# ShudaLi/rgbd_pose_estimation

Hardware: AMD Instinct MI355X
Metric: correspondence-residuals/sec (higher is better)
Workload: dtype f32; 1 GPU; configs[1]: 640x480 dense depth, 307200 3D-3D corr, point-to-point GN step (K1 normal eq + host 6x6 solve + SE3 exp) over inlier mask; corr_rank0=307200, global_corr=307200, collective=none, rccl_ranks=0, rccl_verified=False, repeats=1

## Files before the change

rgbd_pose_estimation_amd/csrc/rpe_normal_eq.hip:

```cpp
#include "rpe_residuals.hpp"

namespace rpe {

__global__ void gn_update_probe_kernel(const double* __restrict__ rec, double* __restrict__ pose, double* __restrict__ step_ok,
                                       double rel_floor) {
  __shared__ double s_rec[32];
  __shared__ double s_pose[12];
  if (threadIdx.x < 32) s_rec[threadIdx.x] = rec[threadIdx.x];
  if (threadIdx.x < 12) s_pose[threadIdx.x] = pose[threadIdx.x];
  __syncthreads();
  if (threadIdx.x == 0) {
    double step = 0.0;
    const bool ok = gn_solve_update<0>(s_rec, s_pose, &step, rel_floor);
    step_ok[0] = step; step_ok[1] = ok ? 1.0 : 0.0;
    if (ok) for (int k = 0; k < 12; k++) pose[k] = s_pose[k];
  }
}
hipError_t launch_gn_update_probe(const double* d_rec, double* d_pose, double* d_step_ok, double pivot_floor, hipStream_t s) {
  hipLaunchKernelGGL(gn_update_probe_kernel, dim3(1), dim3(64), 0, s, d_rec, d_pose, d_step_ok, pivot_floor);
  return hipGetLastError();
}

template <class T, int KIND, int BLK, bool MASK, bool WEIGHT, bool CLEAN>
__global__ __launch_bounds__(BLK) void normal_eq_kernel(const T* __restrict__ xw, const T* __restrict__ b, const T* __restrict__ c,
// ... 28 lines not shown
#pragma unroll
  for (int k = 0; k < NACC; k++) carry[k] = V2{T(0), T(0)};
  int carried = 0;
  int64_t g = (int64_t)blockIdx.x * BLK + threadIdx.x;
  V a0, a1, a2, b0, b1, b2, c0, c1, c2;
  short m[P];
  T wv[P];
  if (g < full) {
    a0 = xw4[3 * g]; a1 = xw4[3 * g + 1]; a2 = xw4[3 * g + 2];
    b0 = b4[3 * g]; b1 = b4[3 * g + 1]; b2 = b4[3 * g + 2];
    if (KIND == KIND_P2PLANE) { c0 = c4[3 * g]; c1 = c4[3 * g + 1]; c2 = c4[3 * g + 2]; }
    if (MASK) load_mask_full(mask, g, m);
    if (WEIGHT) load_weight_full(weight, g, wv);
    pin16(a0); pin16(a1); pin16(a2); pin16(b0); pin16(b1); pin16(b2);
    if (KIND == KIND_P2PLANE) { pin16(c0); pin16(c1); pin16(c2); }
  }
#if defined(RPE_STAMPS) && RPE_STAMPS >= 2
  asm volatile("s_waitcnt vmcnt(0)" ::: "memory");
  RPE_STAMP(11);
#endif
  while (g < full) {
    const int64_t gn = g + stride;
    const int64_t gl = gn < full ? gn : g;
    const V na0 = xw4[3 * gl], na1 = xw4[3 * gl + 1], na2 = xw4[3 * gl + 2];
    const V nb0 = b4[3 * gl], nb1 = b4[3 * gl + 1], nb2 = b4[3 * gl + 2];
    V nc0, nc1, nc2;
    if (KIND == KIND_P2PLANE) { nc0 = c4[3 * gl]; nc1 = c4[3 * gl + 1]; nc2 = c4[3 * gl + 2]; }
    short nm[P];
    T nwv[P];
    if (MASK) load_mask_full(mask, gl, nm);
    if (WEIGHT) load_weight_full(weight, gl, nwv);
    __builtin_amdgcn_sched_barrier(0);
    T vw[3 * P], vb[3 * P], vc[3 * P];
    unpack3(a0, a1, a2, vw);
    unpack3(b0, b1, b2, vb);
    if (KIND == KIND_P2PLANE) unpack3(c0, c1, c2, vc);
    pair_group<T, KIND, MASK, WEIGHT, CLEAN, NACC>(pose, vw, vb, vc, m, wv, P, carry);
    if (++carried == kShare) { flush_pairs<T, NACC>(carry, acc); carried = 0; }
    a0 = na0; a1 = na1; a2 = na2; b0 = nb0; b1 = nb1; b2 = nb2;
    if (KIND == KIND_P2PLANE) { c0 = nc0; c1 = nc1; c2 = nc2; }
    __builtin_amdgcn_sched_barrier(0);
    pin16(a0); pin16(a1); pin16(a2); pin16(b0); pin16(b1); pin16(b2);
    if (KIND == KIND_P2PLANE) { pin16(c0); pin16(c1); pin16(c2); }
#pragma unroll
    for (int i = 0; i < P; i++) { if (MASK) m[i] = nm[i]; if (WEIGHT) wv[i] = nwv[i]; }
    g = gn;
  }
  if (blockIdx.x == 0 && threadIdx.x == 0 && full * P < n) {
    T vw[3 * P], vb[3 * P], vc[3 * P];
    short lm[P];
    T lwv[P];
    load_group<T>(xw, full, n, vw);
    load_group<T>(b, full, n, vb);
    if (KIND == KIND_P2PLANE) load_group<T>(c, full, n, vc);
    if (MASK) load_scalars<T, short>(mask, full, n, lm, (short)0);
    if (WEIGHT) load_scalars<T, T>(weight, full, n, lwv, T(0));
    pair_group<T, KIND, MASK, WEIGHT, CLEAN, NACC>(pose, vw, vb, vc, lm, lwv, (int)(n - full * P), carry);
    carried = 1;
  }
  if (carried) flush_pairs<T, NACC>(carry, acc);
  RPE_STAMP(1);
  reduce_and_finish<NACC, kNeLd, KIND == KIND_P2P ? 1 : 0, BLK>(acc, fin);
}

template <class T, int KIND, int BLK, bool MASK, bool WEIGHT, int NREG, int AUTO, bool CLEAN>
__global__ __launch_bounds__(BLK) void normal_eq_resident_kernel(const T* __restrict__ xw, const T* __restrict__ b, const T* __restrict__ c,
                             const short* __restrict__ mask, const T* __restrict__ weight, int64_t n,
                             const unsigned long long* __restrict__ ctl, unsigned long long first_tag, int max_iters, Finish fin) {
  constexpr int P = Pk<T>::P;
  constexpr int NACC = KIND == KIND_P2P ? 17 : 29;
  constexpr bool IN_REGS = NREG > 0;
  constexpr int GPT = IN_REGS ? NREG : 1;
  __shared__ double s_pose[12];
  __shared__ int s_go;
  const int64_t full = n / P, groups = (n + P - 1) / P;
  constexpr bool with_solver = AUTO == 2;
  const int workers = (int)gridDim.x;
  const int64_t stride = (int64_t)workers * BLK;
  const int64_t g0 = (int64_t)blockIdx.x * (BLK * GPT) + threadIdx.x;
  T rw[GPT][3 * P], rb[GPT][3 * P], rc[GPT][3 * P];
  short rm[GPT][P];
  T rwv[GPT][P];
  int rpresent[GPT];
#pragma unroll
  for (int r = 0; r < GPT; r++) {
    rpresent[r] = 0;
    const int64_t g = g0 + (int64_t)r * BLK;
    if (IN_REGS && g < groups) {
      load_any_group<T, KIND, MASK, WEIGHT>(xw, b, c, mask, weight, g, full, n, rw[r], rb[r], rc[r], rm[r], rwv[r]);
      rpresent[r] = g < full ? P : (int)(n - full * P);
    }
  }
#ifdef RPE_SOLVER_DEBUG
  if (with_solver && threadIdx.x == 0) __hip_atomic_store(solver_pose_area(fin, workers, NACC) + 32 + blockIdx.x, wall_clock64(), __ATOMIC_RELAXED, __HIP_MEMORY_SCOPE_AGENT);
#endif
  constexpr bool autonomous = AUTO != 0;
  double tol = 0.0;
  if (autonomous) {
    if (threadIdx.x < 12) s_pose[threadIdx.x] = fin.gn_pose[threadIdx.x];
    tol = fin.gn->tol;
    __syncthreads();
  }
  for (int it = 1; it <= max_iters; it++) {
    if (!autonomous && resident_wait_pose<BLK>(ctl, first_tag + (unsigned long long)it, s_pose, &s_go,
        fin.pose_wait_ticks) != 1) return;
    if (with_solver && it > 1 && solver_wait_pose<BLK>(solver_pose_area(fin, workers, NACC), first_tag + (unsigned long long)it, s_pose, &s_go, it == 2 ? kSolverMeetTicks : 200000000ull) != 0) return;
#ifdef RPE_STAMPS
    const bool stamp_it = it == 1000;
    if (stamp_it) RPE_STAMP(0);
#endif
    PoseK<double> pose;
#pragma unroll
    for (int k = 0; k < 9; k++) pose.R[k] = s_pose[k];
#pragma unroll
    for (int k = 0; k < 3; k++) pose.t[k] = s_pose[9 + k];
    double acc[NACC];
#pragma unroll
    for (int k = 0; k < NACC; k++) acc[k] = 0.0;
    if (IN_REGS) {
#pragma unroll
      for (int r = 0; r < GPT; r++)
        if (rpresent[r] > 0) normal_eq_group<T, KIND, MASK, WEIGHT, NACC, CLEAN>(pose, rw[r], rb[r], rc[r], rm[r], rwv[r], rpresent[r], acc);
    } else {
      for (int64_t g = g0; g < groups; g += stride) {
        T vw[3 * P], vb[3 * P], vc[3 * P];
        short mm[P];
        T ww[P];
        load_any_group<T, KIND, MASK, WEIGHT>(xw, b, c, mask, weight, g, full, n, vw, vb, vc, mm, ww);
        normal_eq_group<T, KIND, MASK, WEIGHT, NACC, CLEAN>(pose, vw, vb, vc, mm, ww, g < full ? P : (int)(n - full * P), acc);
      }
    }
#ifdef RPE_STAMPS
    if (stamp_it) RPE_STAMP(1);
#endif
#ifndef RPE_STAMPS
    const bool stamp_it = false;
#endif
    if (with_solver) { solver_send_sums<NACC, BLK>(acc, fin, first_tag + (unsigned long long)it); continue; }
    if (autonomous) {
      if (resident_auto_stage<NACC, BLK>(acc, fin, first_tag + (unsigned long long)it, it, max_iters, tol, s_pose,
          stamp_it) != 0) return;
      continue;
    }
    if (!resident_cross_stage<NACC, BLK>(acc, fin, first_tag + (unsigned long long)it, fin.seq + (unsigned long long)it,
        stamp_it)) return;
  }
}

#ifdef RPE_STAMPS
}
extern "C" int rpe_debug_read_stamps(unsigned long long* out, int nwords) {
  if (nwords > 4096 * 16) nwords = 4096 * 16;
  if (hipDeviceSynchronize() != hipSuccess) return -1;
  if (hipMemcpyFromSymbol(out, HIP_SYMBOL(rpe::g_stamps), (size_t)nwords * 8) != hipSuccess) return -1;
  static unsigned long long zeros[4096 * 16];
  return hipMemcpyToSymbol(HIP_SYMBOL(rpe::g_stamps), zeros, sizeof(zeros)) == hipSuccess ? 0 : -1;
}
namespace rpe {
#endif

template <int MODE>
__global__ __launch_bounds__(64) void chain_finish_kernel(const double* __restrict__ runs, const double* __restrict__ pose_in, GnState* st,
                                                          double rel_floor, double* __restrict__ h_pairs, unsigned long long seq) {
  __shared__ double f_tot[32];
  __shared__ double f_pose[12];
  __shared__ double f_out[16];
  if (threadIdx.x < 12) f_pose[threadIdx.x] = pose_in[threadIdx.x];
  if (threadIdx.x < 32) {
    double t = 0.0;
#pragma unroll
    for (int r = 0; r < kRunSlots; r++) t += runs[r * kRunLd + threadIdx.x];
    f_tot[threadIdx.x] = t;
  }
  __syncthreads();
  if (threadIdx.x == 0) {
    double step = st->step;
    bool ok = st->status == 0;
    if (!st->done) ok = gn_solve_update<MODE>(f_tot, f_pose, &step, rel_floor);
    for (int k = 0; k < 12; k++) f_out[k] = f_pose[k];
    f_out[12] = step; f_out[13] = st->done ? st->cost : record_entry<MODE>(f_tot, 27); f_out[14] = (double)(st->iters + (st->done ? 0 : 1));
    f_out[15] = ok ? 0.0 : 1.0;
  }
  __syncthreads();
  if (threadIdx.x < 16) store_tagged_pair(h_pairs, threadIdx.x, f_out[threadIdx.x], seq);
}
hipError_t launch_chain_finish(int kind, const double* d_runs, const double* d_pose, GnState* d_state, double pivot_floor, double* h_pairs,
                               unsigned long long seq, hipStream_t s) {
  if (kind == KIND_P2P) hipLaunchKernelGGL((chain_finish_kernel<1>), dim3(1), dim3(64), 0, s, d_runs, d_pose, d_state, pivot_floor, h_pairs, seq);
  else hipLaunchKernelGGL((chain_finish_kernel<0>), dim3(1), dim3(64), 0, s, d_runs, d_pose, d_state, pivot_floor, h_pairs, seq);
  return hipGetLastError();
}

template <class T, int KIND, int BLK>
static void normal_eq_launch(const DeviceArrays& A, int flags, const PoseK<double>& pose, const ReduceTarget& rt, hipStream_t s,
                             hipEvent_t ev0, hipEvent_t ev1) {
  const T* xw = (const T*)A.a[0];
  const T* b = (const T*)((KIND == KIND_BEARING || KIND == KIND_REPROJ) ? A.a[2] : A.a[1]);
  const T* c = (const T*)A.a[4];
  const int mod = (KIND == KIND_BEARING || KIND == KIND_REPROJ) ? 0 : 1;
  const short* mask = (flags & F_USE_MASK) ? A.mask[mod] : nullptr;
  const T* weight = (flags & F_USE_WEIGHT) ? (const T*)A.weight[mod] : nullptr;
  const int G = reduce_grid(A.n, Pk<T>::P, rt.max_blocks, BLK);
  const Finish fin = make_finish(rt);
#define RPE_NE_LAUNCH2(M, W, C) RPE_LAUNCH_EV((normal_eq_kernel<T, KIND, BLK, M, W, C>), dim3(G), dim3(BLK), 0, s, ev0, ev1, xw, b, c, mask, weight, A.n, pose, fin)
#define RPE_NE_LAUNCH(M, W) do { if constexpr (sizeof(T) == 4) { if (rt.clean) { RPE_NE_LAUNCH2(M, W, true); break; } } RPE_NE_LAUNCH2(M, W, false); } while (0)
  if (mask && weight) RPE_NE_LAUNCH(true, true);
  else if (mask) RPE_NE_LAUNCH(true, false);
  else if (weight) RPE_NE_LAUNCH(false, true);
  else RPE_NE_LAUNCH(false, false);
#undef RPE_NE_LAUNCH
#undef RPE_NE_LAUNCH2
}
template <class T>
static hipError_t normal_eq_t(const DeviceArrays& A, int kind, int flags, const double* pose12, const ReduceTarget& rt, hipStream_t s,
                              hipEvent_t ev0, hipEvent_t ev1) {
  const PoseK<double> pose = make_pose<double>(pose12);
  const int blk = (sizeof(T) == 8 && kind != KIND_P2P) ? 256 : pick_block(rt);
  if (kind == KIND_P2P) {
    if (blk == 512) normal_eq_launch<T, KIND_P2P, 512>(A, flags, pose, rt, s, ev0, ev1);
    else normal_eq_launch<T, KIND_P2P, 256>(A, flags, pose, rt, s, ev0, ev1);
  } else if (kind == KIND_P2PLANE) {
    if (blk == 512) { if constexpr (sizeof(T) == 4) normal_eq_launch<T, KIND_P2PLANE, 512>(A, flags, pose, rt, s, ev0, ev1); }
    else normal_eq_launch<T, KIND_P2PLANE, 256>(A, flags, pose, rt, s, ev0, ev1);
  } else if (kind == KIND_BEARING) {
    if (blk == 512) { if constexpr (sizeof(T) == 4) normal_eq_launch<T, KIND_BEARING, 512>(A, flags, pose, rt, s, ev0, ev1); }
    else normal_eq_launch<T, KIND_BEARING, 256>(A, flags, pose, rt, s, ev0, ev1);
  } else if (kind == KIND_REPROJ) {
    if (blk == 512) { if constexpr (sizeof(T) == 4) normal_eq_launch<T, KIND_REPROJ, 512>(A, flags, pose, rt, s, ev0, ev1); }
// ... 130 lines not shown
```

rgbd_pose_estimation_amd/csrc/rpe_residuals.hpp:

```cpp
#pragma once
#include "rpe_reduce.hpp"

namespace rpe {

template <class C> __device__ __forceinline__ void add_row(const C (&J)[6], C r, C w, C (&s)[29]) {
  int k = 0;
#pragma unroll
  for (int a = 0; a < 6; a++) {
    const C wa = w * J[a];
#pragma unroll
    for (int b = a; b < 6; b++) { s[k] = fma(wa, J[b], s[k]); k++; }
    s[21 + a] = fma(wa, r, s[21 + a]);
  }
  s[27] = fma(w * r, r, s[27]);
}
template <class V> __device__ __forceinline__ void add_row2(const V (&J)[6], V r, V w, V (&s)[29]) {
  int k = 0;
#pragma unroll
  for (int a = 0; a < 6; a++) {
    const V wa = w * J[a];
#pragma unroll
    for (int b = a; b < 6; b++) { s[k] = __builtin_elementwise_fma(wa, J[b], s[k]); k++; }
    s[21 + a] = __builtin_elementwise_fma(wa, r, s[21 + a]);
  }
// ... 107 lines not shown
  w = ok ? w : C(0);
  n1 = ok ? (C)fma(pxd, (double)bz, -(double)bx * pzd) : C(0);
  n2 = ok ? (C)fma(pyd, (double)bz, -(double)by * pzd) : C(0);
  px = ok ? (C)pxd : C(0); py = ok ? (C)pyd : C(0); pz = ok ? (C)pzd : C(1);
  bzs = ok ? bz : C(1);
}
template <class C>
__device__ __forceinline__ void reproj_pair(const PoseK<double>& T, const C (&x)[2], const C (&y)[2], const C (&z)[2], const C (&bx)[2],
                                            const C (&by)[2], const C (&bz)[2], const C (&w)[2], C __attribute__((ext_vector_type(2))) (&s)[29]) {
  typedef C V __attribute__((ext_vector_type(2)));
  C px[2], py[2], pz[2], n1[2], n2[2], bzs[2], wi[2];
#pragma unroll
  for (int e = 0; e < 2; e++) {
    double pxd, pyd, pzd;
    transform<C>(T, x[e], y[e], z[e], pxd, pyd, pzd);
    wi[e] = w[e];
    reproj_prepare<C>(pxd, pyd, pzd, bx[e], by[e], bz[e], wi[e], px[e], py[e], pz[e], n1[e], n2[e], bzs[e]);
  }
  reproj_rows<V>(V{px[0], px[1]}, V{py[0], py[1]}, V{pz[0], pz[1]}, V{n1[0], n1[1]}, V{n2[0], n2[1]}, V{bzs[0], bzs[1]},
                 V{wi[0], wi[1]}, V{wi[0], wi[1]}, s);
}
template <class C>
__device__ __forceinline__ void reproj_point(double pxd, double pyd, double pzd, C bx, C by, C bz, C w, C w_count, C (&s)[29]) {
  C px, py, pz, n1, n2, bzs, wc = w_count;
  reproj_prepare<C>(pxd, pyd, pzd, bx, by, bz, wc, px, py, pz, n1, n2, bzs);
  reproj_rows<C>(px, py, pz, n1, n2, bzs, wc == C(0) ? C(0) : w, wc, s);
}
template <class C>
__device__ __forceinline__ C reproj_residual_norm(double pxd, double pyd, double pzd, C bx, C by, C bz) {
  if (!(pzd > kReprojMinZ && (double)bz > kReprojMinZ)) return C(0);
  const double r1 = pxd / pzd - (double)bx / (double)bz, r2 = pyd / pzd - (double)by / (double)bz;
  return (C)sqrt(r1 * r1 + r2 * r2);
}
template <class C>
__device__ __forceinline__ void bearing_pair(const PoseK<double>& T, const C (&x)[2], const C (&y)[2], const C (&z)[2], const C (&bx)[2],
                                             const C (&by)[2], const C (&bz)[2], const C (&w)[2],
                                             C __attribute__((ext_vector_type(2))) (&s)[29]) {
  typedef C V __attribute__((ext_vector_type(2)));
  const V BX = {bx[0], bx[1]}, BY = {by[0], by[1]}, BZ = {bz[0], bz[1]};
  V e1[3], e2[3];
  tangent_basis<V>(BX, BY, BZ, e1, e2);
  C px[2], py[2], pz[2], d1[2], d2[2];
#pragma unroll
  for (int e = 0; e < 2; e++) {
    double pxd, pyd, pzd;
    transform<C>(T, x[e], y[e], z[e], pxd, pyd, pzd);
    px[e] = (C)pxd; py[e] = (C)pyd; pz[e] = (C)pzd;
    d1[e] = (C)dot_e_p(e1[0][e], e1[1][e], e1[2][e], pxd, pyd, pzd);
    d2[e] = (C)dot_e_p(e2[0][e], e2[1][e], e2[2][e], pxd, pyd, pzd);
  }
  bearing_rows<V>(V{px[0], px[1]}, V{py[0], py[1]}, V{pz[0], pz[1]}, e1, e2, V{d1[0], d1[1]}, V{d2[0], d2[1]}, BX, BY, BZ,
      V{w[0], w[1]},
                  V{w[0], w[1]}, s);
}


template <class V> __device__ __forceinline__ void p2p_accumulate(V px, V py, V pz, V rx, V ry, V rz, V w, V (&s)[17]) {
  const V wpx = w * px, wpy = w * py, wpz = w * pz;
  const V wrx = w * rx, wry = w * ry, wrz = w * rz;
  s[0] += w;
  s[1] += wpx; s[2] += wpy; s[3] += wpz;
  s[4] = __builtin_elementwise_fma(wpx, px, s[4]); s[5] = __builtin_elementwise_fma(wpx, py, s[5]);
  s[6] = __builtin_elementwise_fma(wpx, pz, s[6]); s[7] = __builtin_elementwise_fma(wpy, py, s[7]);
  s[8] = __builtin_elementwise_fma(wpy, pz, s[8]); s[9] = __builtin_elementwise_fma(wpz, pz, s[9]);
  s[10] += wrx; s[11] += wry; s[12] += wrz;
  s[13] += py * wrz - pz * wry;
  s[14] += pz * wrx - px * wrz;
  s[15] += px * wry - py * wrx;
  s[16] = __builtin_elementwise_fma(wrx, rx, __builtin_elementwise_fma(wry, ry, __builtin_elementwise_fma(wrz, rz, s[16])));
}
template <class C>
__device__ __forceinline__ void p2p_pair(const PoseK<double>& T, const C (&x)[2], const C (&y)[2], const C (&z)[2], const C (&cx)[2],
                                         const C (&cy)[2], const C (&cz)[2], const C (&w)[2], C __attribute__((ext_vector_type(2))) (&s)[17]) {
  typedef C V __attribute__((ext_vector_type(2)));
  C px[2], py[2], pz[2], rx[2], ry[2], rz[2];
#pragma unroll
  for (int e = 0; e < 2; e++) {
    double pxd, pyd, pzd;
    transform<C>(T, x[e], y[e], z[e], pxd, pyd, pzd);
    px[e] = (C)pxd; py[e] = (C)pyd; pz[e] = (C)pzd;
    rx[e] = (C)(pxd - (double)cx[e]); ry[e] = (C)(pyd - (double)cy[e]); rz[e] = (C)(pzd - (double)cz[e]);
  }
  p2p_accumulate<V>(V{px[0], px[1]}, V{py[0], py[1]}, V{pz[0], pz[1]}, V{rx[0], rx[1]}, V{ry[0], ry[1]}, V{rz[0], rz[1]}, V{w[0], w[1]}, s);
}

template <class T, int KIND, bool MASK, bool WEIGHT, bool CLEAN, int NS>
__device__ __forceinline__ void pair_group(const PoseK<double>& pose, const T (&vw)[3 * Pk<T>::P], const T (&vb)[3 * Pk<T>::P],
                                           const T (&vc)[3 * Pk<T>::P], const short (&m)[Pk<T>::P], const T (&wv)[Pk<T>::P],
                                           int npresent, T __attribute__((ext_vector_type(2))) (&s2)[NS]) {
  constexpr int P = Pk<T>::P;
  static_assert(NS == (KIND == KIND_P2P ? 17 : 29), "sums per kind");
  static_assert(KIND == KIND_P2P || KIND == KIND_P2PLANE || KIND == KIND_BEARING || KIND == KIND_REPROJ, "residual kinds");
#pragma unroll
  for (int j = 0; j < P / 2; j++) {
    T x[2], y[2], z[2], bx[2], by[2], bz[2], nx[2], ny[2], nz[2], wi[2];
#pragma unroll
    for (int e = 0; e < 2; e++) {
      const int i = 2 * j + e;
      bx[e] = vb[3 * i]; by[e] = vb[3 * i + 1]; bz[e] = vb[3 * i + 2];
      T w = WEIGHT ? wv[i] : T(1);
      if (MASK) w = m[i] == 1 ? w : T(0);
      if (CLEAN) {
        w = i < npresent ? w : T(0);
        x[e] = vw[3 * i]; y[e] = vw[3 * i + 1]; z[e] = vw[3 * i + 2];
        if (KIND == KIND_P2PLANE) { nx[e] = vc[3 * i]; ny[e] = vc[3 * i + 1]; nz[e] = vc[3 * i + 2]; }
      } else {
        w = (i < npresent && !all_nan(bx[e], by[e], bz[e])) ? w : T(0);
        const bool off = w == T(0);
        x[e] = off ? T(0) : vw[3 * i]; y[e] = off ? T(0) : vw[3 * i + 1];
        z[e] = off ? ((KIND == KIND_BEARING || KIND == KIND_REPROJ) ? T(1) : T(0)) : vw[3 * i + 2];
        bx[e] = off ? T(0) : bx[e]; by[e] = off ? T(0) : by[e]; bz[e] = off ? T(1) : bz[e];
        if (KIND == KIND_P2PLANE) { nx[e] = off ? T(0) : vc[3 * i]; ny[e] = off ? T(0) : vc[3 * i + 1];
            nz[e] = off ? T(0) : vc[3 * i + 2]; }
      }
      wi[e] = w;
    }
    if constexpr (KIND == KIND_P2P) p2p_pair<T>(pose, x, y, z, bx, by, bz, wi, s2);
    else if constexpr (KIND == KIND_P2PLANE) p2plane_pair<T>(pose, x, y, z, bx, by, bz, nx, ny, nz, wi, s2);
    else if constexpr (KIND == KIND_BEARING) bearing_pair<T>(pose, x, y, z, bx, by, bz, wi, s2);
    else {
      reproj_pair<T>(pose, x, y, z, bx, by, bz, wi, s2);
      if (CLEAN) {
        typedef T V __attribute__((ext_vector_type(2)));
        const V all = ((V{x[0], x[1]} + V{y[0], y[1]}) + (V{z[0], z[1]} + V{bx[0], bx[1]})) + (V{by[0], by[1]} + V{bz[0], bz[1]});
        s2[27] = __builtin_elementwise_fma(V{T(0), T(0)}, all, s2[27]);
      }
    }
  }
}
template <class T, int NS>
__device__ __forceinline__ void flush_pairs(T __attribute__((ext_vector_type(2))) (&s2)[NS], double (&acc)[NS]) {
  typedef T V __attribute__((ext_vector_type(2)));
#pragma unroll
  for (int k = 0; k < NS; k++) { acc[k] += (double)(s2[k].x + s2[k].y); s2[k] = V{T(0), T(0)}; }
}

template <class T, int KIND, bool MASK, bool WEIGHT, int NACC, bool CLEAN = false>
__device__ __forceinline__ void normal_eq_group(const PoseK<double>& pose, const T (&vw)[3 * Pk<T>::P], const T (&vb)[3 * Pk<T>::P],
                                                const T (&vc)[3 * Pk<T>::P], const short (&m)[Pk<T>::P], const T (&wv)[Pk<T>::P],
                                                int npresent, double (&acc)[NACC]) {
  typedef T V __attribute__((ext_vector_type(2)));
  V s2[NACC];
#pragma unroll
  for (int k = 0; k < NACC; k++) s2[k] = V{T(0), T(0)};
  pair_group<T, KIND, MASK, WEIGHT, CLEAN, NACC>(pose, vw, vb, vc, m, wv, npresent, s2);
  flush_pairs<T, NACC>(s2, acc);
}
constexpr unsigned long long kResidentStop = 1ull << 63;
template <class T, int KIND, bool MASK, bool WEIGHT>
__device__ __forceinline__ void load_any_group(const T* __restrict__ xw, const T* __restrict__ b, const T* __restrict__ c,
                                               const short* __restrict__ mask, const T* __restrict__ weight, int64_t g, int64_t full,
                                               int64_t n, T (&vw)[3 * Pk<T>::P], T (&vb)[3 * Pk<T>::P], T (&vc)[3 * Pk<T>::P],
                                               short (&m)[Pk<T>::P], T (&wv)[Pk<T>::P]) {
  typedef typename Pk<T>::V V;
  if (g < full) {
    const V* xw4 = reinterpret_cast<const V*>(xw);
    const V* b4 = reinterpret_cast<const V*>(b);
    const V x0 = xw4[3 * g], x1 = xw4[3 * g + 1], x2 = xw4[3 * g + 2];
    const V y0 = b4[3 * g], y1 = b4[3 * g + 1], y2 = b4[3 * g + 2];
    unpack3(x0, x1, x2, vw);
    unpack3(y0, y1, y2, vb);
    if (KIND == KIND_P2PLANE) { const V* c4 = reinterpret_cast<const V*>(c);
        const V z0 = c4[3 * g], z1 = c4[3 * g + 1], z2 = c4[3 * g + 2]; unpack3(z0, z1, z2, vc); }
    if (MASK) load_mask_full(mask, g, m);
    if (WEIGHT) load_weight_full(weight, g, wv);
  } else {
// ... 4 lines not shown
    if (WEIGHT) load_scalars<T, T>(weight, g, n, wv, T(0));
  }
}

constexpr int kAutoMaxRunSums = 1024;
__device__ __forceinline__ int resident_judge_pose(unsigned long long w, unsigned long long want) {
  const unsigned int lo = (unsigned int)w, hi = (unsigned int)(w >> 32);
  const unsigned long long ta = ((unsigned long long)__builtin_amdgcn_readlane(hi, 0) << 32) | __builtin_amdgcn_readlane(lo, 0);
  const unsigned long long tb = ((unsigned long long)__builtin_amdgcn_readlane(hi, 15) << 32) | __builtin_amdgcn_readlane(lo, 15);
  if (ta != tb) return 0;
  const unsigned long long num = ta & ~kResidentStop;
  if (num == want) return (ta & kResidentStop) ? 2 : 1;
  return num > want ? 2 : 0;
}
template <int BLK>
__device__ __forceinline__ int resident_wait_pose(const unsigned long long* __restrict__ ctl, unsigned long long want,
                                                  double* __restrict__ s_pose, int* __restrict__ s_go,
                                                  unsigned long long wait_ticks = 200000000ull) {
  if (threadIdx.x < 64) {
    const int lane = threadIdx.x;
    const unsigned long long t0 = wall_clock64();
    int go = 0;
    unsigned long long w = 0;
    for (;;) {
      if (lane < 16) w = __hip_atomic_load(ctl + lane, __ATOMIC_RELAXED, __HIP_MEMORY_SCOPE_SYSTEM);
      if ((go = resident_judge_pose(w, want)) != 0) break;
      if (wall_clock64() - t0 > wait_ticks) { go = 3; break; }
      __builtin_amdgcn_s_sleep(2);
    }
    if (lane >= 1 && lane <= 12) s_pose[lane - 1] = __longlong_as_double((long long)w);
    if (lane == 0) *s_go = go;
  }
  __syncthreads();
  return *s_go;
}
struct RunShape { int run, row, leader, rows, runs, step; };
__device__ __forceinline__ RunShape run_shape(const Finish& fin, int G) {
  RunShape s;
  const int b = (int)blockIdx.x;
  if (fin.stride > 1) {
    const int S = fin.stride < G ? fin.stride : G;
    s.run = b % S; s.row = b / S; s.leader = s.run; s.rows = (G - s.run + S - 1) / S; s.runs = S; s.step = S;
  } else {
    const int R = fin.rows;
    s.run = b / R; s.leader = s.run * R; s.row = b - s.leader; s.rows = min(R, G - s.leader); s.runs = (G + R - 1) / R; s.step = 1;
  }
  return s;
}
template <int NACC, int BLK>
__device__ __forceinline__ bool resident_cross_own(double own, const Finish& fin, unsigned long long tag, unsigned long long seq, bool stamp_it) {
  constexpr int RGN = BLK / NACC;
  __shared__ double g_part[RGN][NACC];
  unsigned long long* gran = reinterpret_cast<unsigned long long*>(fin.partials);
  const RunShape rs = run_shape(fin, (int)gridDim.x);
  const int run = rs.run, leader = rs.leader;
  if ((int)blockIdx.x != leader) {
    const bool withheld = fin.fault_tag != 0 && tag == fin.fault_tag && blockIdx.x + 1 == gridDim.x;
    if (threadIdx.x < NACC && !withheld) store_granule16(gran + 2 * ((size_t)blockIdx.x * NACC + threadIdx.x), own, tag);
#ifdef RPE_STAMPS
    if (stamp_it) RPE_STAMP(2);
#endif
    return true;
  }
  if (threadIdx.x < NACC) g_part[0][threadIdx.x] = own;
#ifdef RPE_STAMPS
  if (stamp_it) RPE_STAMP(2);
#endif
  const int rows = rs.rows;
  const bool lost = collect_rows<NACC, BLK>(gran, (int)gridDim.x, leader, rows, tag, g_part, rs.step);
#ifdef RPE_STAMPS
  if (stamp_it) RPE_STAMP(3);
#endif
  const bool ok = !__syncthreads_or(lost);
#ifdef RPE_STAMPS
  if (stamp_it) RPE_STAMP(4);
#endif
  if (threadIdx.x < NACC) store_tagged_pair(fin.out_host, run * NACC + threadIdx.x,
      ok ? sum_rows_lane<NACC, RGN>(g_part, rows < RGN ? rows : RGN, threadIdx.x) : __longlong_as_double((long long)kLostMarker), seq);
#ifdef RPE_STAMPS
  if (stamp_it) RPE_STAMP(5);
#endif
  return ok;
}
template <int NACC, int BLK>
__device__ __forceinline__ bool resident_cross_stage(const double (&acc)[NACC], const Finish& fin, unsigned long long tag,
                                                     unsigned long long seq, bool stamp_it) {
  constexpr int NW = BLK / 64;
  __shared__ double g_red[NW][NACC];
  const int lane = threadIdx.x & 63, wave = threadIdx.x >> 6;
  wave_reduce_to<NACC>(acc, g_red[wave], lane);
  __syncthreads();
  double own = 0.0;
  if (threadIdx.x < NACC) {
#pragma unroll
    for (int w = 0; w < NW; w++) own += g_red[w][threadIdx.x];
  }
  return resident_cross_own<NACC, BLK>(own, fin, tag, seq, stamp_it);
}

template <int NACC, int BLK>
__device__ __forceinline__ int resident_auto_stage(const double (&acc)[NACC], const Finish& fin, unsigned long long tag, int it,
                                                   int max_iters, double tol, double* __restrict__ s_pose, bool stamp_it = false) {
  constexpr int NW = BLK / 64;
  constexpr int RGN = BLK / NACC;
  constexpr int MODE = NACC == 17 ? 1 : 0;
  __shared__ double a_red[NW][NACC];
  __shared__ double a_part[RGN][NACC];
  __shared__ double a_runs[kAutoMaxRunSums];
  __shared__ double a_tot[32];
  __shared__ double a_step;
  __shared__ int a_ok;
  const int lane = threadIdx.x & 63, wave = threadIdx.x >> 6;
  const int G = (int)gridDim.x;
  const RunShape rs = run_shape(fin, G);
  const int run = rs.run, leader = rs.leader, runs = rs.runs;
  unsigned long long* gran = reinterpret_cast<unsigned long long*>(fin.partials);
  unsigned long long* rrec = gran + 2 * ((size_t)G * NACC + (size_t)(it & 1) * runs * NACC);
  wave_reduce_to<NACC>(acc, a_red[wave], lane);
  __syncthreads();
  if (threadIdx.x < NACC) {
    double own = 0.0;
#pragma unroll
    for (int w = 0; w < NW; w++) own += a_red[w][threadIdx.x];
    if ((int)blockIdx.x != leader) store_granule16(gran + 2 * ((size_t)blockIdx.x * NACC + threadIdx.x), own, tag);
    else a_part[0][threadIdx.x] = own;
  }
#ifdef RPE_STAMPS
  if (stamp_it) RPE_STAMP(2);
#endif
  bool lost = runs * NACC > kAutoMaxRunSums;
  if (!lost && (int)blockIdx.x == leader) {
    const int rows = rs.rows;
    lost = __syncthreads_or(collect_rows<NACC, BLK>(gran, G, leader, rows, tag, a_part, rs.step));
    if (!lost) {
      const double t = sum_rows<NACC, BLK>(a_part, rows < RGN ? rows : RGN);
      if (threadIdx.x < NACC) { if (G == 1) a_runs[threadIdx.x] = t; else store_granule16(rrec + 2 * ((size_t)run * NACC + threadIdx.x), t, tag); }
    }
  }
#ifdef RPE_STAMPS
  if (stamp_it) RPE_STAMP(3);
#endif
  if (!lost && G > 1) {
    const int total = runs * NACC;
    for (int i = threadIdx.x; i < total; i += BLK) {
      const unsigned long long t0 = wall_clock64();
      granule_t q;
      for (unsigned int spins = 1;; spins++) {
        q = load_granule16(rrec + 2 * (size_t)i);
        if ((((unsigned long long)q.w << 32) | q.z) == tag) break;
        if ((spins & 63u) == 0 && wall_clock64() - t0 > 200000000ull) { lost = true; break; }
      }
      a_runs[i] = __longlong_as_double((long long)(((unsigned long long)q.y << 32) | q.x));
    }
  }
  lost = __syncthreads_or(lost);
#ifdef RPE_STAMPS
  if (stamp_it) RPE_STAMP(4);
#endif
  if (threadIdx.x < 64) {
    if (!lost) {
      double t = 0.0;
      if (threadIdx.x < NACC) for (int r = 0; r < runs; r++) t += a_runs[r * NACC + threadIdx.x];
      if (threadIdx.x < 32) a_tot[threadIdx.x] = threadIdx.x < NACC ? t : 0.0;
    }
    __builtin_amdgcn_fence(__ATOMIC_RELEASE, "wavefront");
    __builtin_amdgcn_wave_barrier();
    __builtin_amdgcn_fence(__ATOMIC_ACQUIRE, "wavefront");
#ifdef RPE_STAMPS
    if (stamp_it) RPE_STAMP(5);
#endif
    if (threadIdx.x == 0) {
      double step = 0.0;
      a_ok = !lost && gn_solve_update<MODE>(a_tot, s_pose, &step, fin.pivot_floor) ? 1 : 0;
      a_step = step;
    }
  }
  __syncthreads();
#ifdef RPE_STAMPS
  if (stamp_it) RPE_STAMP(6);
#endif
  const bool ok = a_ok != 0;
  const bool done = !ok || a_step < tol || it >= max_iters;
  if (done && blockIdx.x == 0 && threadIdx.x == 0 && fin.out_host) {
    for (int k = 0; k < 12; k++) __hip_atomic_store(fin.out_host + k, s_pose[k], __ATOMIC_RELAXED, __HIP_MEMORY_SCOPE_SYSTEM);
    __hip_atomic_store(fin.out_host + 12, a_step, __ATOMIC_RELAXED, __HIP_MEMORY_SCOPE_SYSTEM);
    __hip_atomic_store(fin.out_host + 13, lost ? 0.0 : record_entry<MODE>(a_tot, 27), __ATOMIC_RELAXED, __HIP_MEMORY_SCOPE_SYSTEM);
    __hip_atomic_store(fin.out_host + 14, (double)it, __ATOMIC_RELAXED, __HIP_MEMORY_SCOPE_SYSTEM);
    __hip_atomic_store(fin.out_host + 15, ok ? 0.0 : (lost ? 2.0 : 1.0), __ATOMIC_RELAXED, __HIP_MEMORY_SCOPE_SYSTEM);
    __hip_atomic_store(fin.out_host + 16, lost ? 0.0 : record_entry<MODE>(a_tot, 28), __ATOMIC_RELAXED, __HIP_MEMORY_SCOPE_SYSTEM);
    asm volatile("s_waitcnt vmcnt(0)" ::: "memory");
    __hip_atomic_store(reinterpret_cast<unsigned long long*>(fin.out_host + 32), fin.seq, __ATOMIC_RELAXED, __HIP_MEMORY_SCOPE_SYSTEM);
  }
  return lost ? 2 : (done ? 1 : 0);
}

constexpr int kSolverPoseGranules = 14;
constexpr unsigned long long kSolverMeetTicks = 25000000ull;
__device__ __forceinline__ unsigned long long* solver_pose_area(const Finish& fin, int workers, int nacc) {
  return reinterpret_cast<unsigned long long*>(fin.partials) + 2 * ((size_t)(workers + 8) * nacc);
}
template <int BLK>
__device__ __forceinline__ int solver_wait_pose(const unsigned long long* __restrict__ area, unsigned long long want, double* __restrict__ s_pose,
                                                int* __restrict__ s_go, unsigned long long wait_ticks = 200000000ull) {
  if (threadIdx.x < 64) {
    const int lane = threadIdx.x;
    const unsigned long long t0 = wall_clock64();
    granule_t q = {};
    int go = -1;
    for (unsigned int spins = 1;; spins++) {
      bool have = true;
      if (lane < kSolverPoseGranules) {
        q = load_granule16(area + 2 * (size_t)lane);
        have = (((unsigned long long)q.w << 32) | q.z) == want;
      }
      if (__builtin_amdgcn_ballot_w64(!have) == 0) { go = 0; break; }
      if ((spins & 63u) == 0 && wall_clock64() - t0 > wait_ticks) { go = 3; break; }
      __builtin_amdgcn_s_sleep(1);
    }
    const double v = __longlong_as_double((long long)(((unsigned long long)q.y << 32) | q.x));
    if (lane < 12) s_pose[lane] = v;
    if (lane == 13) *s_go = go == 3 ? 3 : (int)v;
  }
  __syncthreads();
  return *s_go;
}
template <int NACC, int BLK>
__device__ __forceinline__ void solver_send_sums(const double (&acc)[NACC], const Finish& fin, unsigned long long tag) {
  constexpr int NW = BLK / 64;
  __shared__ double w_red[NW][NACC];
  const int lane = threadIdx.x & 63, wave = threadIdx.x >> 6;
  unsigned long long* gran = reinterpret_cast<unsigned long long*>(fin.partials);
  wave_reduce_to<NACC>(acc, w_red[wave], lane);
  __syncthreads();
  if (threadIdx.x < NACC) {
    double own = 0.0;
#pragma unroll
    for (int w = 0; w < NW; w++) own += w_red[w][threadIdx.x];
    store_granule16(gran + 2 * ((size_t)blockIdx.x * NACC + threadIdx.x), own, tag);
  }
  __syncthreads();
}
template <int NACC, int BLK>
__device__ __forceinline__ void solver_loop(const Finish& fin, int workers, unsigned long long first_tag, int max_iters) {
  constexpr int RGN = BLK / NACC;
  constexpr int MODE = NACC == 17 ? 1 : 0;
  __shared__ double v_part[RGN][NACC];
  __shared__ double v_tot[32];
  __shared__ double v_pose[12];
  __shared__ double v_step;
  __shared__ int v_code;
  unsigned long long* gran = reinterpret_cast<unsigned long long*>(fin.partials);
  unsigned long long* area = solver_pose_area(fin, workers, NACC);
#ifdef RPE_SOLVER_DEBUG
  const unsigned long long dbg_start = wall_clock64();
#endif
  if (threadIdx.x < 12) v_pose[threadIdx.x] = fin.gn_pose[threadIdx.x];
  const double tol = fin.gn->tol;
  __syncthreads();
  for (int it = 1; it <= max_iters; it++) {
    const unsigned long long tag = first_tag + (unsigned long long)it;
    if (threadIdx.x < NACC) v_part[0][threadIdx.x] = 0.0;
    __syncthreads();
    bool lost = collect_rows<NACC, BLK, 12>(gran, workers, -1, workers + 1, tag, v_part, 1, it <= 2 ? kSolverMeetTicks : 200000000ull);
    lost = __syncthreads_or(lost);
    if (lost && threadIdx.x == 0 && fin.out_host) {
      int missing = 0, lo = workers, hi = -1;
      for (int w = 0; w < workers; w++) {
        const granule_t q = load_granule16(gran + 2 * ((size_t)w * NACC + NACC - 1));
        if ((((unsigned long long)q.w << 32) | q.z) != tag) { missing++; lo = w < lo ? w : lo; hi = w; }
      }
#ifdef RPE_SOLVER_DEBUG
      {
        unsigned long long mn = ~0ull, mx = 0; int started = 0;
        for (int w = 0; w < workers; w++) {
          const unsigned long long v = __hip_atomic_load(area + 32 + w, __ATOMIC_RELAXED, __HIP_MEMORY_SCOPE_AGENT);
          if (v > dbg_start - 100000000ull) { started++; mn = v < mn ? v : mn; mx = v > mx ? v : mx; }
        }
        __hip_atomic_store(fin.out_host + 20, (double)started, __ATOMIC_RELAXED, __HIP_MEMORY_SCOPE_SYSTEM);
        __hip_atomic_store(fin.out_host + 21, started ? ((double)mn - (double)dbg_start) * 0.01 : -1.0, __ATOMIC_RELAXED, __HIP_MEMORY_SCOPE_SYSTEM);
        __hip_atomic_store(fin.out_host + 22, started ? ((double)mx - (double)dbg_start) * 0.01 : -1.0, __ATOMIC_RELAXED, __HIP_MEMORY_SCOPE_SYSTEM);
        __hip_atomic_store(fin.out_host + 23, ((double)wall_clock64() - (double)dbg_start) * 0.01, __ATOMIC_RELAXED, __HIP_MEMORY_SCOPE_SYSTEM);
      }
#endif
      __hip_atomic_store(fin.out_host + 17, (double)missing, __ATOMIC_RELAXED, __HIP_MEMORY_SCOPE_SYSTEM);
      __hip_atomic_store(fin.out_host + 18, (double)lo, __ATOMIC_RELAXED, __HIP_MEMORY_SCOPE_SYSTEM);
      __hip_atomic_store(fin.out_host + 19, (double)hi, __ATOMIC_RELAXED, __HIP_MEMORY_SCOPE_SYSTEM);
    }
    const double t = sum_rows<NACC, BLK>(v_part, workers + 1 < RGN ? workers + 1 : RGN);
    if (threadIdx.x < 64) {
      if (threadIdx.x < 32) v_tot[threadIdx.x] = threadIdx.x < NACC ? t : 0.0;
      __builtin_amdgcn_fence(__ATOMIC_RELEASE, "wavefront");
      __builtin_amdgcn_wave_barrier();
      __builtin_amdgcn_fence(__ATOMIC_ACQUIRE, "wavefront");
      if (threadIdx.x == 0) {
        double step = 0.0;
        const bool ok = !lost && gn_solve_update<MODE>(v_tot, v_pose, &step, fin.pivot_floor);
        v_step = step;
        v_code = !ok ? 2 : ((step < tol || it >= max_iters) ? 1 : 0);
      }
      __builtin_amdgcn_fence(__ATOMIC_RELEASE, "wavefront");
      __builtin_amdgcn_wave_barrier();
      __builtin_amdgcn_fence(__ATOMIC_ACQUIRE, "wavefront");
      const int lane = threadIdx.x;
      if (lane == 0 && v_code != 0 && fin.out_host) {
        const bool ok = v_code == 1;
        for (int k = 0; k < 12; k++) __hip_atomic_store(fin.out_host + k, v_pose[k], __ATOMIC_RELAXED, __HIP_MEMORY_SCOPE_SYSTEM);
        __hip_atomic_store(fin.out_host + 12, v_step, __ATOMIC_RELAXED, __HIP_MEMORY_SCOPE_SYSTEM);
        __hip_atomic_store(fin.out_host + 13, lost ? 0.0 : record_entry<MODE>(v_tot, 27), __ATOMIC_RELAXED, __HIP_MEMORY_SCOPE_SYSTEM);
        __hip_atomic_store(fin.out_host + 14, (double)it, __ATOMIC_RELAXED, __HIP_MEMORY_SCOPE_SYSTEM);
        __hip_atomic_store(fin.out_host + 15, ok ? 0.0 : (lost ? 2.0 : 1.0), __ATOMIC_RELAXED, __HIP_MEMORY_SCOPE_SYSTEM);
        __hip_atomic_store(fin.out_host + 16, lost ? 0.0 : record_entry<MODE>(v_tot, 28), __ATOMIC_RELAXED, __HIP_MEMORY_SCOPE_SYSTEM);
        asm volatile("s_waitcnt vmcnt(0)" ::: "memory");
        __hip_atomic_store(reinterpret_cast<unsigned long long*>(fin.out_host + 32), fin.seq, __ATOMIC_RELAXED, __HIP_MEMORY_SCOPE_SYSTEM);
        asm volatile("s_waitcnt vmcnt(0)" ::: "memory");
      }
      __builtin_amdgcn_fence(__ATOMIC_RELEASE, "wavefront");
      __builtin_amdgcn_wave_barrier();
      if (lane < kSolverPoseGranules) {
        const double v = lane < 12 ? v_pose[lane] : (lane == 12 ? v_step : (double)v_code);
        store_granule16(area + 2 * (size_t)lane, v, tag + 1);
// ... 17 lines not shown
```

Baseline: 45.72 billion correspondence-residuals/s.

## Precompute sanitised weights and pose-invariant weight sum once in resident P2P kernel

For the register-resident f32 point-to-point path, the mask/weight/NaN sanitisation is done once before the iteration loop, and the weight sum (accumulator 0, which does not depend on the pose) is reduced once and reused every iteration. The per-iteration loop then uses a dedicated packed-f32 accumulation over register groups and a 16-wide wave reduce-scatter in place of reducing all 17 sums. This cuts per-iteration ALU and reduction work, at the cost of extra registers for the precomputed weights and some code duplication across three staging paths.

Measured after the change: 48.23 billion correspondence-residuals/s, median of 6. +5.5%, better.

```diff
diff --git a/rgbd_pose_estimation_amd/csrc/rpe_normal_eq.hip b/rgbd_pose_estimation_amd/csrc/rpe_normal_eq.hip
--- a/rgbd_pose_estimation_amd/csrc/rpe_normal_eq.hip
+++ b/rgbd_pose_estimation_amd/csrc/rpe_normal_eq.hip
@@ -134,6 +134,9 @@
   short rm[GPT][P];
   T rwv[GPT][P];
   int rpresent[GPT];
+  constexpr bool ONCE = IN_REGS && KIND == KIND_P2P && sizeof(T) == 4;
+  T rwt[GPT][P];
+  double sum0 = 0.0;
 #pragma unroll
   for (int r = 0; r < GPT; r++) {
     rpresent[r] = 0;
@@ -141,8 +144,15 @@
     if (IN_REGS && g < groups) {
       load_any_group<T, KIND, MASK, WEIGHT>(xw, b, c, mask, weight, g, full, n, rw[r], rb[r], rc[r], rm[r], rwv[r]);
       rpresent[r] = g < full ? P : (int)(n - full * P);
+    } else if (ONCE) {
+#pragma unroll
+      for (int k = 0; k < 3 * P; k++) { rw[r][k] = T(0); rb[r][k] = T(0); }
+#pragma unroll
+      for (int k = 0; k < P; k++) { rm[r][k] = 0; rwv[r][k] = T(0); }
     }
-  }
+    if constexpr (ONCE) resident_sanitise<T, MASK, WEIGHT, CLEAN>(rw[r], rb[r], rm[r], rwv[r], rpresent[r], rwt[r]);
+  }
+  if constexpr (ONCE) sum0 = resident_weight_sum<T, GPT, BLK>(rwt);
 #ifdef RPE_SOLVER_DEBUG
   if (with_solver && threadIdx.x == 0) __hip_atomic_store(solver_pose_area(fin, workers, NACC) + 32 + blockIdx.x, wall_clock64(), __ATOMIC_RELAXED, __HIP_MEMORY_SCOPE_AGENT);
 #endif
@@ -167,6 +177,23 @@
 #pragma unroll
     for (int k = 0; k < 3; k++) pose.t[k] = s_pose[9 + k];
     double acc[NACC];
+    if constexpr (ONCE) {
+      p2p_groups_in_regs<T, GPT>(pose, rw, rb, rwt, acc);
+#ifdef RPE_STAMPS
+      if (stamp_it) RPE_STAMP(1);
+#endif
+#ifndef RPE_STAMPS
+      const bool stamp_it = false;
+#endif
+      if (with_solver) { solver_send_sums<NACC, BLK, true>(acc, fin, first_tag + (unsigned long long)it, sum0); continue; }
+      if (autonomous) {
+        if (resident_auto_stage<NACC, BLK, true>(acc, fin, first_tag + (unsigned long long)it, it, max_iters, tol, s_pose,
+            stamp_it, sum0) != 0) return;
+        continue;
+      }
+      if (!resident_cross_stage<NACC, BLK, true>(acc, fin, first_tag + (unsigned long long)it, fin.seq + (unsigned long long)it,
+          stamp_it, sum0)) return;
+    } else {
 #pragma unroll
     for (int k = 0; k < NACC; k++) acc[k] = 0.0;
     if (IN_REGS) {
@@ -196,6 +223,7 @@
     }
     if (!resident_cross_stage<NACC, BLK>(acc, fin, first_tag + (unsigned long long)it, fin.seq + (unsigned long long)it,
         stamp_it)) return;
+    }
   }
 }
 
diff --git a/rgbd_pose_estimation_amd/csrc/rpe_residuals.hpp b/rgbd_pose_estimation_amd/csrc/rpe_residuals.hpp
--- a/rgbd_pose_estimation_amd/csrc/rpe_residuals.hpp
+++ b/rgbd_pose_estimation_amd/csrc/rpe_residuals.hpp
@@ -213,6 +213,84 @@
     rx[e] = (C)(pxd - (double)cx[e]); ry[e] = (C)(pyd - (double)cy[e]); rz[e] = (C)(pzd - (double)cz[e]);
   }
   p2p_accumulate<V>(V{px[0], px[1]}, V{py[0], py[1]}, V{pz[0], pz[1]}, V{rx[0], rx[1]}, V{ry[0], ry[1]}, V{rz[0], rz[1]}, V{w[0], w[1]}, s);
+}
+template <class T, int NG>
+__device__ __forceinline__ void p2p_groups_in_regs(const PoseK<double>& pose, const T (&vw)[NG][3 * Pk<T>::P],
+                                                   const T (&vb)[NG][3 * Pk<T>::P], const T (&w)[NG][Pk<T>::P], double (&acc)[17]) {
+  constexpr int P = Pk<T>::P;
+  typedef T V __attribute__((ext_vector_type(2)));
+  acc[0] = 0.0;
+#pragma unroll
+  for (int r = 0; r < NG; r++) {
+    V s2[17];
+#pragma unroll
+    for (int k = 0; k < 17; k++) s2[k] = V{T(-0.0), T(-0.0)};
+#pragma unroll
+    for (int j = 0; j < P / 2; j++) {
+      T x[2], y[2], z[2], bx[2], by[2], bz[2], wi[2];
+#pragma unroll
+      for (int e = 0; e < 2; e++) {
+        const int i = 2 * j + e;
+        x[e] = vw[r][3 * i]; y[e] = vw[r][3 * i + 1]; z[e] = vw[r][3 * i + 2];
+        bx[e] = vb[r][3 * i]; by[e] = vb[r][3 * i + 1]; bz[e] = vb[r][3 * i + 2];
+        wi[e] = w[r][i];
+      }
+      p2p_pair<T>(pose, x, y, z, bx, by, bz, wi, s2);
+      if (j == 0) {
+#pragma unroll
+        for (int k = 1; k < 17; k++) asm("" : "+v"(s2[k]));
+      }
+    }
+#pragma unroll
+    for (int k = 1; k < 17; k++) {
+      T h = s2[k].x + s2[k].y;
+      asm("" : "+v"(h));
+      if (r == 0) acc[k] = (double)h; else acc[k] += (double)h;
+    }
+  }
+}
+template <class T, bool MASK, bool WEIGHT, bool CLEAN>
+__device__ __forceinline__ void resident_sanitise(T (&vw)[3 * Pk<T>::P], T (&vb)[3 * Pk<T>::P], const short (&m)[Pk<T>::P],
+                                                  const T (&wv)[Pk<T>::P], int npresent, T (&w)[Pk<T>::P]) {
+#pragma unroll
+  for (int i = 0; i < Pk<T>::P; i++) {
+    T wi = WEIGHT ? wv[i] : T(1);
+    if (MASK) wi = m[i] == 1 ? wi : T(0);
+    if (CLEAN) {
+      wi = i < npresent ? wi : T(0);
+    } else {
+      wi = (i < npresent && !all_nan(vb[3 * i], vb[3 * i + 1], vb[3 * i + 2])) ? wi : T(0);
+      if (wi == T(0)) { vw[3 * i] = vw[3 * i + 1] = vw[3 * i + 2] = T(0); vb[3 * i] = vb[3 * i + 1] = T(0); vb[3 * i + 2] = T(1); }
+    }
+    w[i] = wi;
+  }
+}
+template <class T, int NG, int BLK>
+__device__ __forceinline__ double resident_weight_sum(const T (&w)[NG][Pk<T>::P]) {
+  constexpr int P = Pk<T>::P, NW = BLK / 64;
+  __shared__ double s_w[NW];
+  double t = 0.0;
+#pragma unroll
+  for (int r = 0; r < NG; r++) {
+    T lo = T(0), hi = T(0);
+#pragma unroll
+    for (int j = 0; j < P / 2; j++) { lo += w[r][2 * j]; hi += w[r][2 * j + 1]; }
+    t += (double)(lo + hi);
+  }
+  t = wave_sum_to_lane63(t);
+  if ((threadIdx.x & 63) == 63) s_w[threadIdx.x >> 6] = t;
+  __syncthreads();
+  double all = 0.0;
+#pragma unroll
+  for (int k = 0; k < NW; k++) all += s_w[k];
+  return all;
+}
+__device__ __forceinline__ void wave_reduce_tail16(const double (&acc)[17], double* __restrict__ out, int lane) {
+  double v[16];
+#pragma unroll
+  for (int k = 0; k < 16; k++) v[k] = acc[k + 1];
+  const double r = wave_reduce_scatter16(v, lane);
+  if ((lane & 3) == 0) out[1 + ((lane >> 2) & 15)] = r;
 }
 
 template <class T, int KIND, bool MASK, bool WEIGHT, bool CLEAN, int NS>
@@ -383,25 +461,28 @@
 #endif
   return ok;
 }
-template <int NACC, int BLK>
+template <int NACC, int BLK, bool SUM0 = false>
 __device__ __forceinline__ bool resident_cross_stage(const double (&acc)[NACC], const Finish& fin, unsigned long long tag,
-                                                     unsigned long long seq, bool stamp_it) {
+                                                     unsigned long long seq, bool stamp_it, double sum0 = 0.0) {
   constexpr int NW = BLK / 64;
   __shared__ double g_red[NW][NACC];
   const int lane = threadIdx.x & 63, wave = threadIdx.x >> 6;
-  wave_reduce_to<NACC>(acc, g_red[wave], lane);
+  if constexpr (SUM0) wave_reduce_tail16(acc, g_red[wave], lane);
+  else wave_reduce_to<NACC>(acc, g_red[wave], lane);
   __syncthreads();
   double own = 0.0;
   if (threadIdx.x < NACC) {
 #pragma unroll
     for (int w = 0; w < NW; w++) own += g_red[w][threadIdx.x];
   }
+  if (SUM0 && threadIdx.x == 0) own = sum0;
   return resident_cross_own<NACC, BLK>(own, fin, tag, seq, stamp_it);
 }
 
-template <int NACC, int BLK>
+template <int NACC, int BLK, bool SUM0 = false>
 __device__ __forceinline__ int resident_auto_stage(const double (&acc)[NACC], const Finish& fin, unsigned long long tag, int it,
-                                                   int max_iters, double tol, double* __restrict__ s_pose, bool stamp_it = false) {
+                                                   int max_iters, double tol, double* __restrict__ s_pose, bool stamp_it = false,
+                                                   double sum0 = 0.0) {
   constexpr int NW = BLK / 64;
   constexpr int RGN = BLK / NACC;
   constexpr int MODE = NACC == 17 ? 1 : 0;
@@ -417,12 +498,14 @@
   const int run = rs.run, leader = rs.leader, runs = rs.runs;
   unsigned long long* gran = reinterpret_cast<unsigned long long*>(fin.partials);
   unsigned long long* rrec = gran + 2 * ((size_t)G * NACC + (size_t)(it & 1) * runs * NACC);
-  wave_reduce_to<NACC>(acc, a_red[wave], lane);
+  if constexpr (SUM0) wave_reduce_tail16(acc, a_red[wave], lane);
+  else wave_reduce_to<NACC>(acc, a_red[wave], lane);
   __syncthreads();
   if (threadIdx.x < NACC) {
     double own = 0.0;
 #pragma unroll
     for (int w = 0; w < NW; w++) own += a_red[w][threadIdx.x];
+    if (SUM0 && threadIdx.x == 0) own = sum0;
     if ((int)blockIdx.x != leader) store_granule16(gran + 2 * ((size_t)blockIdx.x * NACC + threadIdx.x), own, tag);
     else a_part[0][threadIdx.x] = own;
   }
@@ -525,18 +608,20 @@
   __syncthreads();
   return *s_go;
 }
-template <int NACC, int BLK>
-__device__ __forceinline__ void solver_send_sums(const double (&acc)[NACC], const Finish& fin, unsigned long long tag) {
+template <int NACC, int BLK, bool SUM0 = false>
+__device__ __forceinline__ void solver_send_sums(const double (&acc)[NACC], const Finish& fin, unsigned long long tag, double sum0 = 0.0) {
   constexpr int NW = BLK / 64;
   __shared__ double w_red[NW][NACC];
   const int lane = threadIdx.x & 63, wave = threadIdx.x >> 6;
   unsigned long long* gran = reinterpret_cast<unsigned long long*>(fin.partials);
-  wave_reduce_to<NACC>(acc, w_red[wave], lane);
+  if constexpr (SUM0) wave_reduce_tail16(acc, w_red[wave], lane);
+  else wave_reduce_to<NACC>(acc, w_red[wave], lane);
   __syncthreads();
   if (threadIdx.x < NACC) {
     double own = 0.0;
 #pragma unroll
     for (int w = 0; w < NW; w++) own += w_red[w][threadIdx.x];
+    if (SUM0 && threadIdx.x == 0) own = sum0;
     store_granule16(gran + 2 * ((size_t)blockIdx.x * NACC + threadIdx.x), own, tag);
   }
   __syncthreads();
```
